# enoche/MMRec

Hardware: AMD Instinct MI355X
Metric: GCN-layer edges/sec (3-layer user-item CSR SpMM, d=64, fp32) (higher is better)
Workload: dtype f32

## Files before the change

include/mmrec_hip.h:

```cpp
#ifndef MMREC_HIP_H
#define MMREC_HIP_H

#include <stddef.h>
#include <stdint.h>

#ifdef __cplusplus
extern "C" {
#endif

#define MMREC_ABI_VERSION 16
#define MMREC_EMB_DIM 64

#define MMREC_ERR_BAD_ARG 10001
#define MMREC_ERR_UNSUPPORTED 10002

typedef void* mmrec_stream_t;

int mmrec_abi_version(void);
const char* mmrec_error_string(int err);

#ifndef MMREC_SPMM_CHUNK
#define MMREC_SPMM_CHUNK 512
#endif
#define MMREC_SPMM_LONG_ROW_DEFAULT 32

int mmrec_spmm_csr_f32(const int32_t* rowptr, const int32_t* colidx, const float* vals,
                       const float* X, float* Y, const float* Z, const float* acc_in, float* acc_out,
                       int32_t n_rows, int32_t d, float alpha, float beta, float acc_scale,
                       int32_t long_row_threshold, const int32_t* long_rows,
                       const int32_t* long_chunk_ptr, int32_t n_long, int32_t n_chunks,
                       float* partials, int32_t* long_tickets, mmrec_stream_t stream);

int mmrec_spmm_rows_f32(const int32_t* rowptr, const int32_t* colidx, const float* vals, const float* X,
                        const float* Z, int32_t z_compact, const int64_t* rows, int32_t n_list, int32_t d,
                        int32_t long_row_threshold, float* Y, mmrec_stream_t stream);
int mmrec_spmm_rows_any_f32(const int32_t* rowptr, const int32_t* colidx, const float* vals, const float* X,
                            const float* Z, int32_t z_compact, const int64_t* rows, int32_t n_list, int32_t d,
                            int32_t long_row_threshold, int32_t max_row_chunks, float* Y, mmrec_stream_t stream);
int mmrec_spmm_push_rows_f32(const int32_t* rowptr, const int32_t* colidx, const float* vals, const float* G,
                             float g_scale, const int64_t* rows, int32_t n_list, int32_t d, float* dX, float* dZ,
                             mmrec_stream_t stream);

int mmrec_spmm_csr_f32_layergcn(const int32_t* rowptr, const int32_t* colidx, const float* vals, const float* X,
                                float* Y, const float* ego, float* scaled, float* w, const float* acc_in,
                                float* acc_out, int32_t n_rows, int32_t d, int32_t long_row_threshold,
                                const int32_t* long_rows, const int32_t* long_chunk_ptr, int32_t n_long,
                                int32_t n_chunks, float* partials, int32_t* long_tickets, mmrec_stream_t stream);
int mmrec_spmm_csr_sched_f32(const int32_t* rowptr, const int32_t* colidx, const float* vals, const float* X, float* Y,
                             const float* Z, const float* acc_in, float* acc_out, int32_t n_rows, int32_t d, float alpha,
                             float beta, float acc_scale, int32_t long_row_threshold, const int32_t* long_rows,
                             const int32_t* long_chunk_ptr, int32_t n_long, int32_t n_chunks, float* partials,
                             int32_t* long_tickets, const int32_t* sched_row, const int32_t* sched_span,
                             const int32_t* sched_col, const float* sched_val, int32_t n_short, mmrec_stream_t stream);
int mmrec_spmm_csr_sched_f32_layergcn(const int32_t* rowptr, const int32_t* colidx, const float* vals, const float* X,
                                      float* Y, const float* ego, float* scaled, float* w, const float* acc_in,
                                      float* acc_out, int32_t n_rows, int32_t d, int32_t long_row_threshold,
                                      const int32_t* long_rows, const int32_t* long_chunk_ptr, int32_t n_long,
                                      int32_t n_chunks, float* partials, int32_t* long_tickets, const int32_t* sched_row,
                                      const int32_t* sched_span, const int32_t* sched_col, const float* sched_val,
                                      int32_t n_short, mmrec_stream_t stream);
int mmrec_spmm_row_keys(const int32_t* rowptr, const int32_t* colidx, const int32_t* col_degree, int32_t n_rows,
                        int32_t long_row_threshold, int32_t key_deg_max, int32_t* key, int32_t* key_degree,
                        mmrec_stream_t stream);

int mmrec_spmm_csr_masked_f32(const int32_t* rowptr, const int32_t* colidx, const float* vals, const float* X, float* Y,
                              const float* Z, const float* acc_in, float* acc_out, int32_t n_rows, int32_t d, float alpha,
                              float beta, float acc_scale, int32_t long_row_threshold, const int32_t* long_rows,
                              const int32_t* long_chunk_ptr, int32_t n_long, int32_t n_chunks, float* partials,
                              int32_t* long_tickets, const uint32_t* keep_bits, float val_scale, mmrec_stream_t stream);
int mmrec_edge_keep_bits(const uint8_t* keep, int64_t n_edges, const int64_t* perm_a, uint32_t* bits_a,
                         const int64_t* perm_b, uint32_t* bits_b, mmrec_stream_t stream);
int mmrec_spmm_plan_count(const int32_t* rowptr_host, int32_t n_rows, int32_t long_row_threshold,
                          int32_t* n_long, int32_t* n_chunks);
int mmrec_spmm_plan_fill(const int32_t* rowptr_host, int32_t n_rows, int32_t long_row_threshold,
                         int32_t* long_rows, int32_t* long_chunk_ptr);

int mmrec_cos_scale_fwd_f32(const float* E, const float* Ego, float* Out, float* w, float* acc,
                            int32_t n_rows, int32_t d, mmrec_stream_t stream);
int mmrec_cos_scale_bwd_f32(const float* dOut, const float* E, const float* Ego, const float* w,
                            float* dE, float* dEgo_accum, int32_t n_rows, int32_t d,
                            mmrec_stream_t stream);

#define MMREC_BPR_LOGSIG 0
#define MMREC_BPR_GAMMA 1

size_t mmrec_bpr_workspace_bytes(int32_t batch);
int mmrec_bpr_fwd_f32(const float* U, const float* P, const float* N, const int64_t* users,
                      const int64_t* pos, const int64_t* neg, int32_t batch, int32_t d,
                      int32_t variant, float scale, float* loss_out, float* coef, void* workspace,
                      mmrec_stream_t stream);
int mmrec_bpr_bwd_f32(const float* U, const float* P, const float* N, const int64_t* users,
                      const int64_t* pos, const int64_t* neg, int32_t batch, int32_t d,
                      const float* coef, const float* grad_scalar, float scale, float* dU, float* dP,
                      float* dN, mmrec_stream_t stream);

int mmrec_bpr_dots_f32(const float* U, const float* P, const float* N, const int64_t* users,
                       const int64_t* pos, const int64_t* neg, int32_t batch, int32_t d, float* dots,
                       mmrec_stream_t stream);
int mmrec_bpr_loss_from_dots_f32(const float* dots, int32_t batch, int32_t variant, float scale,
                                 float* loss_out, float* coef, void* workspace, mmrec_stream_t stream);

int mmrec_gather_sqnorm_fwd_f32(const float* E, const int64_t* ids, int32_t batch, int32_t d,
                                float* out, void* workspace, mmrec_stream_t stream);
int mmrec_gather_scale_add_bwd_f32(const float* E, const int64_t* ids, int32_t batch, int32_t d,
                                   const float* coef_scalar, float* dE, mmrec_stream_t stream);
#define MMREC_ROWS_REG_MAX_TERMS 6
size_t mmrec_rows_reg_workspace_bytes(int32_t n_terms, int32_t max_batch);
int mmrec_rows_reg_fwd_f32(const float* const* E, const int64_t* const* ids, const int32_t* batch, int32_t n_terms, int32_t d,
                           int32_t mode, float scale, float* out, float* coef, void* workspace, mmrec_stream_t stream);
int mmrec_rows_reg_bwd_f32(const float* const* E, const int64_t* const* ids, const int32_t* batch, int32_t n_terms, int32_t d,
                           const float* coef, const float* g, float* const* dE, mmrec_stream_t stream);

#define MMREC_BPR_MAX_TERMS 4
size_t mmrec_bpr_multi_workspace_bytes(int32_t n_terms, int32_t batch);
int mmrec_bpr_multi_fwd_f32(const float* U, const int64_t* users, const float* const* I, const int64_t* const* pos,
                            const int64_t* const* neg, const float* w, int32_t n_terms, int32_t batch, int32_t d, int32_t variant,
// ... 271 lines not shown
```

mmrec_amd/_lib.py:

```python
from __future__ import annotations

import ctypes
import os
from ctypes import c_char_p, c_float, c_int32, c_int64, c_size_t, c_uint64, c_void_p

import torch

_PKG = os.path.dirname(os.path.abspath(__file__))
LIB_PATH = os.environ.get("MMREC_HIP_LIB") or os.path.join(_PKG, "lib", "libmmrec_hip.so")
ABI_VERSION = 16

_P = c_void_p

SIGNATURES = {
    "mmrec_abi_version": (c_int32, []),
    "mmrec_error_string": (c_char_p, [c_int32]),
    "mmrec_spmm_csr_f32": (c_int32, [_P, _P, _P, _P, _P, _P, _P, _P, c_int32, c_int32, c_float,
                                     c_float, c_float, c_int32, _P, _P, c_int32, c_int32, _P, _P, _P]),
    "mmrec_spmm_csr_f32_layergcn": (c_int32, [_P, _P, _P, _P, _P, _P, _P, _P, _P, _P, c_int32, c_int32, c_int32,
                                              _P, _P, c_int32, c_int32, _P, _P, _P]),
    "mmrec_spmm_csr_sched_f32": (c_int32, [_P, _P, _P, _P, _P, _P, _P, _P, c_int32, c_int32, c_float,
                                           c_float, c_float, c_int32, _P, _P, c_int32, c_int32, _P, _P,
                                           _P, _P, _P, _P, c_int32, _P]),
    "mmrec_spmm_csr_sched_f32_layergcn": (c_int32, [_P, _P, _P, _P, _P, _P, _P, _P, _P, _P, c_int32, c_int32, c_int32,
                                                    _P, _P, c_int32, c_int32, _P, _P, _P, _P, _P, _P, c_int32, _P]),
    "mmrec_spmm_csr_masked_f32": (c_int32, [_P, _P, _P, _P, _P, _P, _P, _P, c_int32, c_int32, c_float,
                                            c_float, c_float, c_int32, _P, _P, c_int32, c_int32, _P, _P, _P, c_float, _P]),
    "mmrec_edge_keep_bits": (c_int32, [_P, c_int64, _P, _P, _P, _P, _P]),
    "mmrec_spmm_row_keys": (c_int32, [_P, _P, _P, c_int32, c_int32, c_int32, _P, _P, _P]),
    "mmrec_spmm_plan_count": (c_int32, [_P, c_int32, c_int32, _P, _P]),
    "mmrec_spmm_plan_fill": (c_int32, [_P, c_int32, c_int32, _P, _P]),
    "mmrec_cos_scale_fwd_f32": (c_int32, [_P, _P, _P, _P, _P, c_int32, c_int32, _P]),
    "mmrec_cos_scale_bwd_f32": (c_int32, [_P, _P, _P, _P, _P, _P, c_int32, c_int32, _P]),
    "mmrec_bpr_workspace_bytes": (c_size_t, [c_int32]),
    "mmrec_bpr_fwd_f32": (c_int32, [_P, _P, _P, _P, _P, _P, c_int32, c_int32, c_int32, c_float, _P,
                                    _P, _P, _P]),
    "mmrec_spmm_rows_f32": (c_int32, [_P, _P, _P, _P, _P, c_int32, _P, c_int32, c_int32, c_int32, _P, _P]),
    "mmrec_spmm_rows_any_f32": (c_int32, [_P, _P, _P, _P, _P, c_int32, _P, c_int32, c_int32, c_int32, c_int32, _P, _P]),
    "mmrec_spmm_push_rows_f32": (c_int32, [_P, _P, _P, _P, c_float, _P, c_int32, c_int32, _P, _P, _P]),
    "mmrec_bpr_dots_f32": (c_int32, [_P, _P, _P, _P, _P, _P, c_int32, c_int32, _P, _P]),
    "mmrec_bpr_loss_from_dots_f32": (c_int32, [_P, c_int32, c_int32, c_float, _P, _P, _P, _P]),
    "mmrec_bpr_bwd_f32": (c_int32, [_P, _P, _P, _P, _P, _P, c_int32, c_int32, _P, _P, c_float, _P, _P,
                                    _P, _P]),
    "mmrec_gather_sqnorm_fwd_f32": (c_int32, [_P, _P, c_int32, c_int32, _P, _P, _P]),
    "mmrec_gather_scale_add_bwd_f32": (c_int32, [_P, _P, c_int32, c_int32, _P, _P, _P]),
    "mmrec_infonce_workspace_bytes": (c_size_t, [c_int32]),
    "mmrec_infonce_fwd_f32": (c_int32, [_P, _P, _P, c_int32, c_int32, c_float, _P, _P, _P]),
    "mmrec_infonce_bwd_f32": (c_int32, [_P, c_int32, c_int32, c_float, _P, _P, _P, _P, _P]),
    "mmrec_linear_workspace_bytes": (c_size_t, [c_int32, c_int32, c_int32]),
    "mmrec_linear_fwd_f32": (c_int32, [_P, _P, _P, _P, c_int32, c_int32, c_int32, _P, _P]),
    "mmrec_linear_fwd_split_f32": (c_int32, [_P, _P, _P, _P, c_int32, c_int32, c_int32, _P, _P]),
    "mmrec_linear_bwd_split_workspace_bytes": (c_size_t, [c_int32, c_int32, c_int32]),
    "mmrec_linear_bwd_split_f32": (c_int32, [_P, _P, _P, _P, _P, _P, c_int32, c_int32, c_int32, _P, _P]),
    "mmrec_linear_bwd_w_f32": (c_int32, [_P, _P, _P, _P, c_int32, c_int32, c_int32, _P, _P]),
    "mmrec_linear_bwd_x_f32": (c_int32, [_P, _P, _P, c_int32, c_int32, c_int32, _P]),
    "mmrec_linear_rows_workspace_bytes": (c_size_t, [c_int32, c_int32, c_int32]),
    "mmrec_linear_rows_fwd_f32": (c_int32, [_P, c_int64, _P, _P, _P, _P, c_int32, c_int32, c_int32, c_int32, _P, _P]),
    "mmrec_linear_rows_bwd_f32": (c_int32, [_P, _P, c_int64, _P, _P, _P, _P, _P, c_int32, c_int32, c_int32, _P, _P]),
    "mmrec_edge_dot_f32": (c_int32, [_P, c_int64, _P, c_int64, _P, _P, c_int64, c_int32, _P, _P]),
    "mmrec_edge_dot_bwd_f32": (c_int32, [_P, _P, c_int64, _P, c_int64, _P, _P, c_int64, c_int32, _P, _P, _P]),
    "mmrec_segment_softmax_group_max": (c_int32, []),
    "mmrec_segment_softmax_f32": (c_int32, [_P, c_int32, _P, _P, c_int32, _P, c_int64, c_float, _P, _P]),
    "mmrec_segment_softmax_bwd_f32": (c_int32, [_P, c_int32, _P, _P, c_int32, _P, _P, c_int64, _P, _P]),
    "mmrec_edge_attention_group_max": (c_int32, []),
    "mmrec_edge_attention_f32": (c_int32, [_P, c_int32, _P, _P, _P, c_int32, _P, c_int64, _P, c_int64, c_int32, c_int64, c_float,
                                           _P, _P, _P]),
    "mmrec_edge_attention_bwd_f32": (c_int32, [_P, c_int32, _P, _P, _P, c_int32, _P, _P, _P, _P, c_int32, _P, c_int64, _P, c_int64,
                                               _P, _P, _P, _P, c_int32, c_int64, _P, _P, _P, _P, _P]),
    "mmrec_neighbor_max_group_max": (c_int32, []),
    "mmrec_neighbor_max_f32": (c_int32, [_P, c_int32, _P, _P, _P, c_int32, _P, c_int64, c_int32, c_int64, _P, _P, _P]),
    "mmrec_neighbor_max_bwd_f32": (c_int32, [_P, c_int32, _P, _P, _P, c_int32, _P, c_int64, _P, c_int32, c_int64, _P, _P, _P]),
    "mmrec_score_lse_split_cols": (c_int32, [c_int32, c_int32, c_int32]),
    "mmrec_score_lse_workspace_bytes": (c_size_t, [c_int32, c_int32, c_int32]),
    "mmrec_score_lse_f32": (c_int32, [_P, _P, c_int32, c_int32, c_int32, c_float, _P, _P, _P]),
    "mmrec_score_lse_bwd_f32": (c_int32, [_P, _P, c_int32, c_int32, c_int32, c_float, _P, _P, _P, _P, _P, _P]),
    "mmrec_hyper_rows_per_block": (c_int32, [c_int64]),
    "mmrec_hyper_workspace_bytes": (c_size_t, [c_int64, c_int64, c_int32]),
    "mmrec_hyper_assign_fwd_f32": (c_int32, [_P, _P, _P, c_int64, c_int32, c_float, c_float, _P, _P, _P]),
# ... 120 lines not shown
```

mmrec_amd/csrc/spmm.hip:

```cpp
#include "common.h"
#include "spmm_narrow.h"

#ifndef MMREC_SPMM_RPG
#define MMREC_SPMM_RPG(n_rows) ((n_rows) <= (1 << 18) ? 1 : 4)
#endif

namespace {

__device__ __forceinline__ void st_coherent(float4* p, float4 v) {
    unsigned long long* q = reinterpret_cast<unsigned long long*>(p);
    const unsigned long long lo = ((unsigned long long)__float_as_uint(v.y) << 32) | __float_as_uint(v.x);
    const unsigned long long hi = ((unsigned long long)__float_as_uint(v.w) << 32) | __float_as_uint(v.z);
    __hip_atomic_store(q, lo, __ATOMIC_RELAXED, __HIP_MEMORY_SCOPE_AGENT);
    __hip_atomic_store(q + 1, hi, __ATOMIC_RELAXED, __HIP_MEMORY_SCOPE_AGENT);
}
__device__ __forceinline__ float4 ld_coherent(const float4* p) {
    unsigned long long* q = reinterpret_cast<unsigned long long*>(const_cast<float4*>(p));
    const unsigned long long lo = __hip_atomic_load(q, __ATOMIC_RELAXED, __HIP_MEMORY_SCOPE_AGENT);
    const unsigned long long hi = __hip_atomic_load(q + 1, __ATOMIC_RELAXED, __HIP_MEMORY_SCOPE_AGENT);
    return make_float4(__uint_as_float((unsigned)lo), __uint_as_float((unsigned)(lo >> 32)),
                       __uint_as_float((unsigned)hi), __uint_as_float((unsigned)(hi >> 32)));
}

struct RowEpilogue {
    const float* Z;
    float* Y;
    const float* acc_in;
    float* acc_out;
    float alpha, beta, acc_scale;
    const float* ego;
    float* scaled;
    float* w_out;
};

struct RowSchedule {
    const int32_t* row;
    const int2* span;
    const int32_t* col;
    const float* val;
    int n_short;
};

template <int DCH, bool LG>
__device__ __forceinline__ void store_row(const RowEpilogue& ep, int row, int lane16, const float4 (&sum)[DCH]) {
    if (DCH == 1 && LG) {
        const size_t off = (size_t)row * 16 + lane16;
        const float4 y = f4_scale(ep.alpha, sum[0]);
        const float4 g = reinterpret_cast<const float4*>(ep.ego)[off];
        const float dot = row16_sum(f4_dot(y, g));
        const float ne = fmaxf(sqrtf(row16_sum(f4_dot(y, y))), 1e-8f);
        const float ng = fmaxf(sqrtf(row16_sum(f4_dot(g, g))), 1e-8f);
        const float w = dot / (ne * ng);
        const float4 o = f4_scale(w, y);
        if (ep.Y) reinterpret_cast<float4*>(ep.Y)[off] = y;
        reinterpret_cast<float4*>(ep.scaled)[off] = o;
        if (lane16 == 0) ep.w_out[row] = w;
        if (ep.acc_out)
            reinterpret_cast<float4*>(ep.acc_out)[off] =
                ep.acc_in ? f4_add(reinterpret_cast<const float4*>(ep.acc_in)[off], o) : o;
        return;
    }
#pragma unroll
    for (int ch = 0; ch < DCH; ++ch) {
        const size_t off = (size_t)row * (16 * DCH) + ch * 16 + lane16;
        float4 y = f4_scale(ep.alpha, sum[ch]);
        if (ep.Z) y = f4_fma(ep.beta, reinterpret_cast<const float4*>(ep.Z)[off], y);
        if (ep.Y) reinterpret_cast<float4*>(ep.Y)[off] = y;
        if (ep.acc_out) {
            const float4 a = reinterpret_cast<const float4*>(ep.acc_in)[off];
            reinterpret_cast<float4*>(ep.acc_out)[off] = f4_scale(ep.acc_scale, f4_add(a, y));
        }
    }
}

template <int DCH>
__device__ __forceinline__ void gather_span(const int32_t* __restrict__ colidx,
                                            const float* __restrict__ vals,
                                            const float4* __restrict__ X4, int s, int e, int lane16,
                                            float4 (&acc)[DCH]) {
    constexpr int NB = DCH == 1 ? 8 : (DCH <= 2 ? 4 : (DCH <= 4 ? 2 : 1));
    for (int base = s; base < e; base += 16) {
        const int k = base + lane16;
        int c = 0;
        float v = 0.f;
        if (k < e) {
            c = colidx[k];
            v = vals[k];
        }
        const int cnt = min(16, e - base);
        for (int j0 = 0; j0 < cnt; j0 += NB) {
            float4 x[NB][DCH];
            float vv[NB];
#pragma unroll
            for (int u = 0; u < NB; ++u) {
                const int j = j0 + u;
                const int cj = __shfl(c, j, 16);
                vv[u] = __shfl(v, j, 16);
#pragma unroll
                for (int ch = 0; ch < DCH; ++ch)
                    x[u][ch] = (j < cnt) ? X4[(size_t)cj * (16 * DCH) + ch * 16 + lane16] : f4_zero();
            }
#pragma unroll
            for (int u = 0; u < NB; ++u)
#pragma unroll
                for (int ch = 0; ch < DCH; ++ch) acc[ch] = f4_fma(vv[u], x[u][ch], acc[ch]);
        }
    }
}

template <int DCH, bool COHERENT, bool LG>
__device__ __forceinline__ void reduce_long_row(const float* __restrict__ partials, int c0, int c1, int row,
                                                const RowEpilogue& ep, float4 (*red)[16 * DCH]) {
    const int lane16 = threadIdx.x & 15, g = threadIdx.x >> 4;
#pragma unroll
    for (int ch = 0; ch < DCH; ++ch) {
        float4 t = f4_zero();
        for (int c = c0 + g; c < c1; c += 16) {
            const float4* src = reinterpret_cast<const float4*>(partials) + (size_t)c * (16 * DCH) + ch * 16 + lane16;
            t = f4_add(t, COHERENT ? ld_coherent(src) : *src);
        }
        red[g][ch * 16 + lane16] = t;
    }
    __syncthreads();
    if (g == 0) {
        float4 r[DCH];
#pragma unroll
        for (int ch = 0; ch < DCH; ++ch) {
            r[ch] = red[0][ch * 16 + lane16];
#pragma unroll
            for (int k = 1; k < 16; ++k) r[ch] = f4_add(r[ch], red[k][ch * 16 + lane16]);
        }
        store_row<DCH, LG>(ep, row, lane16, r);
    }
}

template <int DCH, bool LG, bool SCHED>
__global__ __launch_bounds__(256) void spmm_rows_kernel(
    const int32_t* __restrict__ rowptr, const int32_t* __restrict__ colidx,
    const float* __restrict__ vals, const float* __restrict__ X, RowEpilogue ep, int n_rows,
    int long_t, int rows_per_group, const int32_t* __restrict__ long_rows,
    const int32_t* __restrict__ long_chunk_ptr, int n_long, int n_chunks,
    float* __restrict__ partials, int32_t* __restrict__ tickets, RowSchedule sched) {
    __shared__ float4 red[16][16 * DCH];
    __shared__ int s_last;
    const int lane16 = threadIdx.x & 15;
    const int g = threadIdx.x >> 4;
    const float4* X4 = reinterpret_cast<const float4*>(X);
    if ((int)blockIdx.x < n_chunks) {
        const int chunk = blockIdx.x;
        int lo = 0, hi = n_long;
        while (hi - lo > 1) {
            const int mid = (lo + hi) >> 1;
            if (long_chunk_ptr[mid] <= chunk) lo = mid; else hi = mid;
        }
        const int row = long_rows[lo];
        const int cs = rowptr[row] + (chunk - long_chunk_ptr[lo]) * MMREC_SPMM_CHUNK;
        const int ce = min(cs + MMREC_SPMM_CHUNK, rowptr[row + 1]);
        float4 acc[DCH];
#pragma unroll
        for (int ch = 0; ch < DCH; ++ch) acc[ch] = f4_zero();
        for (int base = cs + g * 16; base < ce; base += 256)
            gather_span<DCH>(colidx, vals, X4, base, min(base + 16, ce), lane16, acc);
#pragma unroll
        for (int ch = 0; ch < DCH; ++ch) red[g][ch * 16 + lane16] = acc[ch];
        __syncthreads();
        if (g == 0) {
            float4 t[DCH];
#pragma unroll
            for (int ch = 0; ch < DCH; ++ch) {
                t[ch] = red[0][ch * 16 + lane16];
#pragma unroll
                for (int i = 1; i < 16; ++i) t[ch] = f4_add(t[ch], red[i][ch * 16 + lane16]);
            }
            if (long_chunk_ptr[lo + 1] - long_chunk_ptr[lo] == 1) {
                store_row<DCH, LG>(ep, row, lane16, t);
            } else {
#pragma unroll
                for (int ch = 0; ch < DCH; ++ch) {
                    float4* dst = reinterpret_cast<float4*>(partials) + (size_t)chunk * (16 * DCH) + ch * 16 + lane16;
                    if (tickets) st_coherent(dst, t[ch]); else *dst = t[ch];
                }
            }
        }
        const int c0 = long_chunk_ptr[lo], c1 = long_chunk_ptr[lo + 1];
        if (!tickets || c1 - c0 == 1) return;
        if (threadIdx.x < 64) {
            __atomic_signal_fence(__ATOMIC_SEQ_CST);
            __builtin_amdgcn_s_waitcnt(0);
            __atomic_signal_fence(__ATOMIC_SEQ_CST);
            __builtin_amdgcn_fence(__ATOMIC_RELEASE, "workgroup");
            if (threadIdx.x == 0)
                s_last = __hip_atomic_fetch_add(tickets + lo, 1, __ATOMIC_RELAXED, __HIP_MEMORY_SCOPE_AGENT) == c1 - c0 - 1;
        }
        __syncthreads();
        if (!s_last) return;
        __builtin_amdgcn_fence(__ATOMIC_ACQUIRE, "workgroup");
        reduce_long_row<DCH, true, LG>(partials, c0, c1, row, ep, red);
        if (threadIdx.x == 0) __hip_atomic_store(tickets + lo, 0, __ATOMIC_RELAXED, __HIP_MEMORY_SCOPE_AGENT);
        return;
    }
    if (SCHED) {
        const int slot0 = ((int)blockIdx.x - n_chunks) * 16 * rows_per_group + g;
#pragma unroll 1
        for (int i = 0; i < rows_per_group; ++i) {
            const int slot = slot0 + i * 16;
            if (slot >= sched.n_short) break;
            const int row = sched.row[slot];
            const int2 se = sched.span[slot];
            float4 acc[DCH];
#pragma unroll
            for (int ch = 0; ch < DCH; ++ch) acc[ch] = f4_zero();
            gather_span<DCH>(sched.col, sched.val, X4, se.x, se.y, lane16, acc);
            store_row<DCH, LG>(ep, row, lane16, acc);
        }
        return;
    }
    const int row0 = ((int)blockIdx.x - n_chunks) * 16 * rows_per_group + g;
#pragma unroll 1
    for (int i = 0; i < rows_per_group; ++i) {
        const int row = row0 + i * 16;
        if (row >= n_rows) break;
        const int s = rowptr[row], e = rowptr[row + 1];
        if (e - s > long_t) continue;
        float4 acc[DCH];
#pragma unroll
        for (int ch = 0; ch < DCH; ++ch) acc[ch] = f4_zero();
        gather_span<DCH>(colidx, vals, X4, s, e, lane16, acc);
        store_row<DCH, LG>(ep, row, lane16, acc);
    }
}

template <int DCH, bool LG>
__global__ __launch_bounds__(256) void spmm_long_reduce_kernel(
    const int32_t* __restrict__ long_rows, const int32_t* __restrict__ long_chunk_ptr, int n_long,
    const float* __restrict__ partials, RowEpilogue ep) {
    __shared__ float4 red[16][16 * DCH];
    const int i = blockIdx.x;
    const int c0 = long_chunk_ptr[i], c1 = long_chunk_ptr[i + 1];
    if (c1 - c0 <= 1) return;
    reduce_long_row<DCH, false, LG>(partials, c0, c1, long_rows[i], ep, red);
}

template <int DCH, bool LG = false, bool SCHED = false>
void launch_spmm(hipStream_t s, int blocks, int nch, const int32_t* rowptr, const int32_t* colidx,
                 const float* vals, const float* X, const RowEpilogue& ep, int n_rows, int long_t,
                 int rows_per_group, const int32_t* long_rows, const int32_t* long_chunk_ptr, int n_long,
                 float* partials, int32_t* tickets, const RowSchedule& sched = RowSchedule{}) {
    if (blocks + nch > 0)
        hipLaunchKernelGGL((spmm_rows_kernel<DCH, LG, SCHED>), dim3(blocks + nch), dim3(256), 0, s, rowptr, colidx, vals, X,
                           ep, n_rows, long_t, rows_per_group, long_rows, long_chunk_ptr, n_long, nch, partials, tickets,
                           sched);
    if (!tickets && n_long > 0 && nch > n_long)
        hipLaunchKernelGGL((spmm_long_reduce_kernel<DCH, LG>), dim3(n_long), dim3(256), 0, s, long_rows,
                           long_chunk_ptr, n_long, partials, ep);
}

template <int DCH>
__device__ __forceinline__ void gather_span_masked(const int32_t* __restrict__ colidx, const float* __restrict__ vals,
                                                   const uint32_t* __restrict__ keep_bits, float val_scale,
                                                   const float4* __restrict__ X4, int s, int e, int lane16,
                                                   float4 (&acc)[DCH]) {
    constexpr int NB = DCH == 1 ? 8 : (DCH <= 2 ? 4 : (DCH <= 4 ? 2 : 1));
    const int gshift = threadIdx.x & 48;
    for (int base = s; base < e; base += 16) {
        const int k = base + lane16;
        int c = 0;
        float v = 0.f;
        bool kept = false;
        if (k < e) {
            kept = (keep_bits[k >> 5] >> (k & 31)) & 1u;
            c = colidx[k];
            v = vals[k] * val_scale;
        }
        unsigned m = (unsigned)(__ballot(kept) >> gshift) & 0xffffu;
        while (m) {
            float4 x[NB][DCH];
            float vv[NB];
#pragma unroll
            for (int u = 0; u < NB; ++u) {
                const bool on = m != 0;
                const int j = on ? __ffs(m) - 1 : 0;
                m &= m - 1;
                const int cj = __shfl(c, j, 16);
                const float vj = __shfl(v, j, 16);
                vv[u] = on ? vj : 0.f;
#pragma unroll
                for (int ch = 0; ch < DCH; ++ch)
                    x[u][ch] = on ? X4[(size_t)cj * (16 * DCH) + ch * 16 + lane16] : f4_zero();
            }
#pragma unroll
            for (int u = 0; u < NB; ++u)
#pragma unroll
                for (int ch = 0; ch < DCH; ++ch) acc[ch] = f4_fma(vv[u], x[u][ch], acc[ch]);
        }
    }
}

template <int DCH>
__global__ __launch_bounds__(256) void spmm_rows_masked_kernel(
    const int32_t* __restrict__ rowptr, const int32_t* __restrict__ colidx, const float* __restrict__ vals,
    const uint32_t* __restrict__ keep_bits, float val_scale, const float* __restrict__ X, RowEpilogue ep, int n_rows,
    int long_t, int rows_per_group, const int32_t* __restrict__ long_rows, const int32_t* __restrict__ long_chunk_ptr,
    int n_long, int n_chunks, float* __restrict__ partials, int32_t* __restrict__ tickets) {
    __shared__ float4 red[16][16 * DCH];
    __shared__ int s_last;
    const int lane16 = threadIdx.x & 15;
// ... 356 lines not shown
    if (n_long > 0 && (!long_rows || !long_chunk_ptr || !partials || n_chunks <= 0))
        return MMREC_ERR_BAD_ARG;
    if (!sched_args_ok(sched_row, sched_span, sched_col, sched_val, n_short, n_rows)) return MMREC_ERR_BAD_ARG;
    if (Y == X || acc_out == X) return MMREC_ERR_BAD_ARG;
    RowEpilogue ep{Z, Y, acc_in, acc_out, alpha, Z ? beta : 0.f, acc_scale, nullptr, nullptr, nullptr};
    const RowSchedule sched{sched_row, reinterpret_cast<const int2*>(sched_span), sched_col, sched_val, n_short};
    hipStream_t s = mmrec_stream(stream);
    const int rows_per_group = MMREC_SPMM_RPG(n_rows);
    const int blocks = (n_short + 16 * rows_per_group - 1) / (16 * rows_per_group);
    const int long_t = n_long > 0 ? long_row_threshold : INT32_MAX;
    const int nch = n_long > 0 ? n_chunks : 0;
    int32_t* tickets = n_long > 0 ? long_tickets : nullptr;
#define MMREC_SPMM_CASE(D)                                                                                      \
    case D:                                                                                                     \
        launch_spmm<D, false, true>(s, blocks, nch, rowptr, colidx, vals, X, ep, n_rows, long_t, rows_per_group, \
                                    long_rows, long_chunk_ptr, n_long, partials, tickets, sched);               \
        break;
    switch (d / MMREC_EMB_DIM) {
        MMREC_SPMM_CASE(1) MMREC_SPMM_CASE(2) MMREC_SPMM_CASE(3) MMREC_SPMM_CASE(4) MMREC_SPMM_CASE(5)
        MMREC_SPMM_CASE(6)
    }
#undef MMREC_SPMM_CASE
    MMREC_RETURN_LAUNCH_STATUS();
}

extern "C" int mmrec_spmm_csr_sched_f32_layergcn(const int32_t* rowptr, const int32_t* colidx, const float* vals,
                                                 const float* X, float* Y, const float* ego, float* scaled, float* w,
                                                 const float* acc_in, float* acc_out, int32_t n_rows, int32_t d,
                                                 int32_t long_row_threshold, const int32_t* long_rows,
                                                 const int32_t* long_chunk_ptr, int32_t n_long, int32_t n_chunks,
                                                 float* partials, int32_t* long_tickets, const int32_t* sched_row,
                                                 const int32_t* sched_span, const int32_t* sched_col,
                                                 const float* sched_val, int32_t n_short, mmrec_stream_t stream) {
    if (d != MMREC_EMB_DIM) return MMREC_ERR_UNSUPPORTED;
    if (n_rows < 0 || n_long < 0 || n_chunks < 0 || long_row_threshold < 0) return MMREC_ERR_BAD_ARG;
    if (n_rows == 0) return 0;
    if (!rowptr || !X || !ego || !scaled || !w) return MMREC_ERR_BAD_ARG;
    if (n_long > 0 && (!long_rows || !long_chunk_ptr || !partials || n_chunks <= 0)) return MMREC_ERR_BAD_ARG;
    if (!sched_args_ok(sched_row, sched_span, sched_col, sched_val, n_short, n_rows)) return MMREC_ERR_BAD_ARG;
    if (Y == X || scaled == X || acc_out == X) return MMREC_ERR_BAD_ARG;
    RowEpilogue ep{nullptr, Y, acc_in, acc_out, 1.f, 0.f, 1.f, ego, scaled, w};
    const RowSchedule sched{sched_row, reinterpret_cast<const int2*>(sched_span), sched_col, sched_val, n_short};
    hipStream_t s = mmrec_stream(stream);
    const int rows_per_group = MMREC_SPMM_RPG(n_rows);
    const int blocks = (n_short + 16 * rows_per_group - 1) / (16 * rows_per_group);
    const int long_t = n_long > 0 ? long_row_threshold : INT32_MAX;
    const int nch = n_long > 0 ? n_chunks : 0;
    int32_t* tickets = n_long > 0 ? long_tickets : nullptr;
    launch_spmm<1, true, true>(s, blocks, nch, rowptr, colidx, vals, X, ep, n_rows, long_t, rows_per_group, long_rows,
                               long_chunk_ptr, n_long, partials, tickets, sched);
    MMREC_RETURN_LAUNCH_STATUS();
}

extern "C" int mmrec_spmm_row_keys(const int32_t* rowptr, const int32_t* colidx, const int32_t* col_degree,
                                   int32_t n_rows, int32_t long_row_threshold, int32_t key_deg_max, int32_t* key,
                                   int32_t* key_degree, mmrec_stream_t stream) {
    if (n_rows < 0 || long_row_threshold < 0 || key_deg_max < 0) return MMREC_ERR_BAD_ARG;
    if (n_rows == 0) return 0;
    if (!rowptr || !colidx || !col_degree || !key || !key_degree) return MMREC_ERR_BAD_ARG;
    hipLaunchKernelGGL(spmm_row_keys_kernel, dim3((n_rows + 15) / 16), dim3(256), 0, mmrec_stream(stream), rowptr, colidx,
                       col_degree, n_rows, long_row_threshold, key_deg_max, key, key_degree);
    MMREC_RETURN_LAUNCH_STATUS();
}

extern "C" int mmrec_spmm_plan_count(const int32_t* rowptr_host, int32_t n_rows,
                                     int32_t long_row_threshold, int32_t* n_long, int32_t* n_chunks) {
    if (!rowptr_host || !n_long || !n_chunks || n_rows < 0) return MMREC_ERR_BAD_ARG;
    int32_t nl = 0, nc = 0;
    for (int32_t r = 0; r < n_rows; ++r) {
        const int32_t deg = rowptr_host[r + 1] - rowptr_host[r];
        if (deg > long_row_threshold) {
            ++nl;
            nc += (deg + MMREC_SPMM_CHUNK - 1) / MMREC_SPMM_CHUNK;
        }
    }
    *n_long = nl;
    *n_chunks = nc;
    return 0;
}

extern "C" int mmrec_spmm_plan_fill(const int32_t* rowptr_host, int32_t n_rows,
                                    int32_t long_row_threshold, int32_t* long_rows,
                                    int32_t* long_chunk_ptr) {
    if (!rowptr_host || !long_rows || !long_chunk_ptr || n_rows < 0) return MMREC_ERR_BAD_ARG;
    int32_t nl = 0, nc = 0;
    for (int32_t r = 0; r < n_rows; ++r) {
        const int32_t deg = rowptr_host[r + 1] - rowptr_host[r];
        if (deg > long_row_threshold) {
            long_rows[nl] = r;
            long_chunk_ptr[nl] = nc;
            ++nl;
            nc += (deg + MMREC_SPMM_CHUNK - 1) / MMREC_SPMM_CHUNK;
        }
    }
    long_chunk_ptr[nl] = nc;
    return 0;
}

extern "C" int mmrec_cos_scale_fwd_f32(const float* E, const float* Ego, float* Out, float* w,
                                       float* acc, int32_t n_rows, int32_t d, mmrec_stream_t stream) {
    if (d != MMREC_EMB_DIM) return MMREC_ERR_UNSUPPORTED;
    if (n_rows < 0 || (n_rows > 0 && (!E || !Ego || !Out || !w))) return MMREC_ERR_BAD_ARG;
    if (n_rows == 0) return 0;
    hipLaunchKernelGGL(cos_scale_fwd_kernel, dim3((n_rows + 15) / 16), dim3(256), 0,
                       mmrec_stream(stream), E, Ego, Out, w, acc, n_rows);
    MMREC_RETURN_LAUNCH_STATUS();
// ... 14 lines not shown
```

mmrec_amd/hip_ops.py:

```python
from __future__ import annotations

import ctypes
import math

import numpy as np
import torch

from . import _lib

EMB_DIM = 64
LINEAR_F16X3_DEFAULT = True
LINEAR_F16X3 = LINEAR_F16X3_DEFAULT
SLICE_WIDTHS = (8, 16, 32)
SPMM_CHUNK = 512
LONG_ROW_DEFAULT = None


def default_long_row_threshold(n_cols):
    import os
    forced = os.environ.get("MMREC_LONG_ROW_THRESHOLD")
    if forced:
        return int(forced)
    return 16 if n_cols <= (1 << 18) else 32

# ... 300 lines not shown
    def __init__(self, g: CsrGraph, reorder, n_left=None):
        if g.n_rows != g.n_cols:
            raise _lib.MMRecHipError("PermutedGraph needs a square graph")
        dev, n = g.rowptr.device, g.n_rows
        idx, val = g.to_coo_host()
        perm = locality_order(g.rowptr_host, idx[1], n, reorder, n_left=n_left)
        self.base, self.reorder = g, reorder
        self.perm = torch.from_numpy(perm).to(dev)
        inv = np.empty(n, dtype=np.int64)
        inv[perm] = np.arange(n, dtype=np.int64)
        self.inv = torch.from_numpy(inv).to(dev)
        self.graph = CsrGraph.from_coo_host(np.stack([perm[idx[0]], perm[idx[1]]]), val, n, n, dev, symmetric=g.symmetric,
                                            long_row_threshold=g.long_row_threshold)
        self.n_rows = self.n_cols = n
        self.nnz = g.nnz

    def to_new(self, X):
        return X.index_select(0, self.inv)

    def to_old(self, Xp):
        return Xp.index_select(0, self.perm)


def spmm_raw(g: CsrGraph, X, Y=None, Z=None, acc_in=None, acc_out=None, alpha=1.0, beta=1.0,
             acc_scale=1.0):
    lib = _lib.load()
    _chk(X, torch.float32, "X", 2)
    d = X.shape[1]
    if (d not in SLICE_WIDTHS and (d % EMB_DIM or d > 6 * EMB_DIM)) or X.shape[0] < g.n_cols:
        raise _lib.MMRecHipError("X must be [>=%d, 64*k <= 384 (or a feature slice of 8 / 16 / 32 columns)], got %s" %
                                 (g.n_cols, tuple(X.shape)))
    for t, nm in ((Y, "Y"), (Z, "Z"), (acc_in, "acc_in"), (acc_out, "acc_out")):
        if t is not None:
            _chk(t, torch.float32, nm, 2)
            if t.shape[0] < g.n_rows or t.shape[1] != d:
                raise _lib.MMRecHipError("%s must be [>=%d, %d]" % (nm, g.n_rows, d))
    sc = g.scheduled(d)
    if sc is not None:
        g.checked(lib.mmrec_spmm_csr_sched_f32(_p(g.rowptr), _p(g.colidx), _p(g.vals), _p(X), _p(Y), _p(Z),
                                               _p(acc_in), _p(acc_out), g.n_rows, d, float(alpha),
                                               float(beta), float(acc_scale), g.long_row_threshold,
                                               _p(g.long_rows), _p(g.long_chunk_ptr), g.n_long, g.n_chunks,
                                               _p(g.partials_for(d)), _p(g.long_tickets), _p(sc["row"]), _p(sc["span"]),
                                               _p(sc["col"]), _p(sc["val"]), sc["n_short"], _stream()), "spmm_csr_sched_f32")
        return Y if Y is not None else acc_out
    g.checked(lib.mmrec_spmm_csr_f32(_p(g.rowptr), _p(g.colidx), _p(g.vals), _p(X), _p(Y), _p(Z),
                                     _p(acc_in), _p(acc_out), g.n_rows, d, float(alpha),
                                     float(beta), float(acc_scale), g.long_row_threshold,
                                     _p(g.long_rows), _p(g.long_chunk_ptr), g.n_long, g.n_chunks,
                                     _p(g.partials_for(d)), _p(g.long_tickets), _stream()), "spmm_csr_f32")
    return Y if Y is not None else acc_out


ROWS_MAX_CHUNKS = 480


def rows_servable(g: CsrGraph, d):
    if d not in SLICE_WIDTHS + (EMB_DIM,):
        return False
    return g.n_chunks == g.n_long or (d == EMB_DIM and g.max_row_chunks <= ROWS_MAX_CHUNKS)


def spmm_rows_raw(g: CsrGraph, X, rows, Z=None, z_compact=False):
    lib = _lib.load()
    _chk(X, torch.float32, "X", 2), _chk(rows, torch.int64, "rows", 1)
    d = X.shape[1]
    if not rows_servable(g, d) or X.shape[0] < g.n_cols:
        raise _lib.MMRecHipError("spmm_rows: graph with multi-chunk rows, or X not [>=%d, 8 / 16 / 32 / 64]" % g.n_cols)
    if Z is not None and (_chk(Z, torch.float32, "Z", 2).shape[0] < (rows.numel() if z_compact else g.n_rows) or Z.shape[1] != d):
        raise _lib.MMRecHipError("Z must be [>=%d, %d]" % (rows.numel() if z_compact else g.n_rows, d))
    Y = torch.empty(rows.numel(), d, dtype=torch.float32, device=X.device)
    long_t = g.long_row_threshold if g.n_long > 0 else 2 ** 31 - 1
    if g.n_chunks == g.n_long:
        _lib.check(lib.mmrec_spmm_rows_f32(_p(g.rowptr), _p(g.colidx), _p(g.vals), _p(X), _p(Z), 1 if z_compact else 0, _p(rows),
                                           rows.numel(), d, long_t, _p(Y), _stream()), "spmm_rows_f32")
    else:
        _lib.check(lib.mmrec_spmm_rows_any_f32(_p(g.rowptr), _p(g.colidx), _p(g.vals), _p(X), _p(Z), 1 if z_compact else 0, _p(rows),
                                               rows.numel(), d, long_t, g.max_row_chunks, _p(Y), _stream()), "spmm_rows_any_f32")
    return Y


def spmm_push_rows_raw(g: CsrGraph, G, rows, dX=None, dZ=None, scale=1.0):
    lib = _lib.load()
    _chk(G, torch.float32, "G", 2), _chk(rows, torch.int64, "rows", 1)
    d = G.shape[1]
    if G.shape[0] != rows.numel() or d not in SLICE_WIDTHS + (EMB_DIM,):
        raise _lib.MMRecHipError("G must be [len(rows), 8 / 16 / 32 / 64]")
    for t, nm, n in ((dX, "dX", g.n_cols), (dZ, "dZ", g.n_rows)):
        if t is not None and (_chk(t, torch.float32, nm, 2).shape[0] < n or t.shape[1] != d):
            raise _lib.MMRecHipError("%s must be [>=%d, %d]" % (nm, n, d))
    _lib.check(lib.mmrec_spmm_push_rows_f32(_p(g.rowptr), _p(g.colidx), _p(g.vals), _p(G), float(scale), _p(rows), rows.numel(),
                                            d, _p(dX), _p(dZ), _stream()), "spmm_push_rows_f32")


class _SpmmRows(torch.autograd.Function):

    @staticmethod
    def forward(ctx, X, Z_rows, g, rows):
        ctx.g, ctx.x_shape, ctx.has_z = g, tuple(X.shape), Z_rows is not None
        ctx.save_for_backward(rows)
        return spmm_rows_raw(g, X.contiguous(), rows, None if Z_rows is None else Z_rows.contiguous(), z_compact=True)

    @staticmethod
    def backward(ctx, dY):
        rows, = ctx.saved_tensors
        dY = dY.contiguous()
# ... 4 lines not shown
        return dX, (dY if ctx.has_z and ctx.needs_input_grad[1] else None), None, None


def spmm_rows(g: CsrGraph, X, rows, Z_rows=None):
    if DETERMINISTIC or isinstance(g, PermutedGraph) or not rows_servable(g, X.shape[1]):
        out = spmm(g, X).index_select(0, rows)
        return out if Z_rows is None else out + Z_rows
    return _SpmmRows.apply(X, Z_rows, g, rows)


class _SpMM(torch.autograd.Function):
    @staticmethod
    def forward(ctx, X, Z, g):
        ctx.g, ctx.has_z, ctx.x_rows = g, Z is not None, X.shape[0]
        X = X.contiguous()
        Y = torch.empty(g.n_rows, X.shape[1], dtype=torch.float32, device=X.device)
        spmm_raw(g, X, Y=Y, Z=None if Z is None else Z.contiguous(), beta=1.0)
        return Y

    @staticmethod
    def backward(ctx, dY):
        dY = dY.contiguous()
        gt = ctx.g.transpose()
        dX = None
        if ctx.needs_input_grad[0]:
            alloc = torch.empty if ctx.x_rows == gt.n_rows else torch.zeros
            dX = alloc(ctx.x_rows, dY.shape[1], dtype=torch.float32, device=dY.device)
            spmm_raw(gt, dY, Y=dX)
        return dX, (dY if ctx.has_z and ctx.needs_input_grad[1] else None), None


def spmm(g: CsrGraph, X, Z=None):
    if isinstance(g, PermutedGraph):
        out = spmm(g.graph, g.to_new(X), None if Z is None else g.to_new(Z))
        return g.to_old(out)
    d = X.shape[1]
    if d % EMB_DIM and d not in SLICE_WIDTHS:
        pad = EMB_DIM - d % EMB_DIM
        Xp = torch.nn.functional.pad(X, (0, pad))
        Zp = None if Z is None else torch.nn.functional.pad(Z, (0, pad))
        return _SpMM.apply(Xp, Zp, g)[:, :d]
    return _SpMM.apply(X, Z, g)


class _LightGCNMean(torch.autograd.Function):

    @staticmethod
    def forward(ctx, E0, g, n_layers):
        ctx.g, ctx.L = g, int(n_layers)
        E0 = E0.contiguous()
        L = ctx.L
        if L == 0:
            return E0.clone()
        acc = torch.empty_like(E0)
        bufs = [torch.empty_like(E0) if L > 1 else None, torch.empty_like(E0) if L > 2 else None]
        cur = E0
        for layer in range(1, L + 1):
            last = layer == L
            Y = None if last else bufs[(layer - 1) % 2]
            spmm_raw(g, cur, Y=Y, acc_in=E0 if layer == 1 else acc, acc_out=acc,
                     acc_scale=1.0 / (L + 1) if last else 1.0)
            cur = Y
        return acc

    @staticmethod
    def backward(ctx, dOut):
        L, gt = ctx.L, ctx.g.transpose()
        dOut = dOut.contiguous()
        if L == 0:
            return dOut, None, None
        s = 1.0 / (L + 1)
        bufs = [torch.empty_like(dOut), torch.empty_like(dOut) if L > 1 else None]
        t = dOut
        for j in range(L):
            out = bufs[j % 2]
            spmm_raw(gt, t, Y=out, Z=dOut, alpha=s if j == 0 else 1.0, beta=s)
            t = out
        return t, None, None


def lightgcn_mean(g, E0, n_layers):
    if isinstance(g, PermutedGraph):
        return g.to_old(_LightGCNMean.apply(g.to_new(E0), g.graph, n_layers))
    return _LightGCNMean.apply(E0, g, n_layers)


def row_blocks_of_one_buffer(ts):
    if any(t is None or not t.is_contiguous() or t.dtype != ts[0].dtype for t in ts):
        return False
    base = ts[0].untyped_storage().data_ptr()
    end = ts[0].data_ptr()
    for t in ts:
        if t.untyped_storage().data_ptr() != base or t.data_ptr() != end:
            return False
        end += t.numel() * t.element_size()
    return end <= base + ts[0].untyped_storage().nbytes()


class _LightGCNMeanParts(torch.autograd.Function):

    @staticmethod
    def forward(ctx, g, n_layers, *parts):
        ctx.sizes = [p.shape[0] for p in parts]
        if row_blocks_of_one_buffer(parts):
            E0 = parts[0].detach().as_strided((sum(ctx.sizes), parts[0].shape[1]), (parts[0].shape[1], 1))
        else:
            E0 = torch.cat([p.detach() for p in parts], dim=0)
        ctx.g, ctx.L = g, int(n_layers)
        out = _LightGCNMean.forward(ctx, E0, g, n_layers)
        return tuple(out.split(ctx.sizes))

    @staticmethod
    def backward(ctx, *grads):
        like = next(x for x in grads if x is not None)
        n, d = sum(ctx.sizes), like.shape[1]
        if row_blocks_of_one_buffer(grads):
            dOut = grads[0].as_strided((n, d), (d, 1))
        else:
            dOut = torch.empty((n, d), dtype=like.dtype, device=like.device)
            for dst, src in zip(dOut.split(ctx.sizes), grads):
                dst.zero_() if src is None else dst.copy_(src)
        t = _LightGCNMean.backward(ctx, dOut)[0]
        return (None, None) + tuple(t.split(ctx.sizes))


def lightgcn_mean_parts(g: CsrGraph, parts, n_layers):
    return _LightGCNMeanParts.apply(g, n_layers, *parts)


ROWS_LAST_LAYER = True


class _LightGCNMeanPartsRows(torch.autograd.Function):

    @staticmethod
    def forward(ctx, g, n_layers, rows, *parts):
        ctx.sizes = [p.shape[0] for p in parts]
        if row_blocks_of_one_buffer(parts):
            E0 = parts[0].detach().as_strided((sum(ctx.sizes), parts[0].shape[1]), (parts[0].shape[1], 1))
        else:
            E0 = torch.cat([p.detach() for p in parts], dim=0)
        ctx.save_for_backward(rows)
        L = int(n_layers)
        if L >= 1 and ROWS_LAST_LAYER and rows_servable(g, E0.shape[1]) and E0.shape[0] == g.n_rows == g.n_cols:
            ctx.g, ctx.L = g, L
            E0 = E0.contiguous()
            cur, acc = E0, E0
            if L > 1:
                acc = torch.empty_like(E0)
                bufs = [torch.empty_like(E0), torch.empty_like(E0) if L > 2 else None]
                for layer in range(1, L):
                    Y = bufs[(layer - 1) % 2]
                    spmm_raw(g, cur, Y=Y, acc_in=E0 if layer == 1 else acc, acc_out=acc, acc_scale=1.0)
                    cur = Y
            return spmm_rows_raw(g, cur, rows, Z=acc) * (1.0 / (L + 1))
        out = _LightGCNMean.forward(ctx, E0, g, n_layers)
        return out.index_select(0, rows)

    @staticmethod
    def backward(ctx, dRows):
        rows, = ctx.saved_tensors
        L, g = ctx.L, ctx.g
        dRows = dRows.contiguous()
        n, d = sum(ctx.sizes), dRows.shape[1]
        s = 1.0 / (L + 1)
        t = torch.zeros((n, d), dtype=dRows.dtype, device=dRows.device)
        if L == 0:
            spmm_push_rows_raw(g, dRows, rows, dZ=t)
            return (None, None, None) + tuple(t.split(ctx.sizes))
        spmm_push_rows_raw(g, dRows, rows, dX=t, dZ=t, scale=s)
        gt = g.transpose()
        for _ in range(1, L):
            out = torch.empty_like(t)
            spmm_raw(gt, t, Y=out)
            spmm_push_rows_raw(g, dRows, rows, dZ=out, scale=s)
            t = out
        return (None, None, None) + tuple(t.split(ctx.sizes))


class _MeanPartsRowsThenItemRows(torch.autograd.Function):

    @staticmethod
    def forward(ctx, g, n_layers, rows, mm, item_rows, b, user_table, item_table):
        import types
        inner = types.SimpleNamespace(saved=None)
        inner.save_for_backward = lambda *t: setattr(inner, 'saved', t)
        at = _LightGCNMeanPartsRows.forward(inner, g, n_layers, rows, user_table, item_table)
        ia = spmm_rows_raw(mm, item_table.detach().contiguous(), item_rows, at[b:].contiguous(), z_compact=True)
        ctx.inner = types.SimpleNamespace(sizes=inner.sizes, g=inner.g, L=inner.L)
        ctx.mm, ctx.b = mm, int(b)
        ctx.save_for_backward(rows, item_rows)
        return at[:b].contiguous(), ia

    @staticmethod
    def backward(ctx, d_user_rows, d_ia):
        rows, item_rows = ctx.saved_tensors
        inner = ctx.inner
        inner.saved_tensors = (rows,)
        d_ia = d_ia.contiguous()
        d_rows = torch.cat((d_user_rows.contiguous(), d_ia), dim=0)
# ... 2232 lines not shown
```

Before: 31.26 billion.

## Defer LightGCN layer-sum accumulation to a final multi-table SpMM epilogue

Adds a layer-sum epilogue for the d=64 SpMM kernels. Instead of reading and writing an accumulator on every layer, the intermediate layers now write only Y, and the last layer's kernel sums up to four saved layer tables plus its own result into the output. In the row-gather path, the tables are summed only for the requested rows. The aim is to cut the per-layer read-modify-write accumulator traffic. In exchange the final layer reads more tables and more intermediate buffers are allocated.

```diff
diff --git a/include/mmrec_hip.h b/include/mmrec_hip.h
--- a/include/mmrec_hip.h
+++ b/include/mmrec_hip.h
@@ -62,6 +62,21 @@
 int mmrec_spmm_row_keys(const int32_t* rowptr, const int32_t* colidx, const int32_t* col_degree, int32_t n_rows,
                         int32_t long_row_threshold, int32_t key_deg_max, int32_t* key, int32_t* key_degree,
                         mmrec_stream_t stream);
+
+int mmrec_spmm_csr_layersum_f32(const int32_t* rowptr, const int32_t* colidx, const float* vals, const float* X, float* Y,
+                                const float* S0, const float* S1, const float* S2, const float* S3, int32_t n_sum,
+                                float* out, int32_t n_rows, int32_t d, float alpha, float acc_scale,
+                                int32_t long_row_threshold, const int32_t* long_rows, const int32_t* long_chunk_ptr,
+                                int32_t n_long, int32_t n_chunks, float* partials, int32_t* long_tickets,
+                                mmrec_stream_t stream);
+int mmrec_spmm_csr_sched_layersum_f32(const int32_t* rowptr, const int32_t* colidx, const float* vals, const float* X,
+                                      float* Y, const float* S0, const float* S1, const float* S2, const float* S3,
+                                      int32_t n_sum, float* out, int32_t n_rows, int32_t d, float alpha, float acc_scale,
+                                      int32_t long_row_threshold, const int32_t* long_rows,
+                                      const int32_t* long_chunk_ptr, int32_t n_long, int32_t n_chunks, float* partials,
+                                      int32_t* long_tickets, const int32_t* sched_row, const int32_t* sched_span,
+                                      const int32_t* sched_col, const float* sched_val, int32_t n_short,
+                                      mmrec_stream_t stream);
 
 int mmrec_spmm_csr_masked_f32(const int32_t* rowptr, const int32_t* colidx, const float* vals, const float* X, float* Y,
                               const float* Z, const float* acc_in, float* acc_out, int32_t n_rows, int32_t d, float alpha,
diff --git a/mmrec_amd/_lib.py b/mmrec_amd/_lib.py
--- a/mmrec_amd/_lib.py
+++ b/mmrec_amd/_lib.py
@@ -24,6 +24,11 @@
                                            _P, _P, _P, _P, c_int32, _P]),
     "mmrec_spmm_csr_sched_f32_layergcn": (c_int32, [_P, _P, _P, _P, _P, _P, _P, _P, _P, _P, c_int32, c_int32, c_int32,
                                                     _P, _P, c_int32, c_int32, _P, _P, _P, _P, _P, _P, c_int32, _P]),
+    "mmrec_spmm_csr_layersum_f32": (c_int32, [_P, _P, _P, _P, _P, _P, _P, _P, _P, c_int32, _P, c_int32, c_int32, c_float,
+                                              c_float, c_int32, _P, _P, c_int32, c_int32, _P, _P, _P]),
+    "mmrec_spmm_csr_sched_layersum_f32": (c_int32, [_P, _P, _P, _P, _P, _P, _P, _P, _P, c_int32, _P, c_int32, c_int32, c_float,
+                                                    c_float, c_int32, _P, _P, c_int32, c_int32, _P, _P,
+                                                    _P, _P, _P, _P, c_int32, _P]),
     "mmrec_spmm_csr_masked_f32": (c_int32, [_P, _P, _P, _P, _P, _P, _P, _P, c_int32, c_int32, c_float,
                                             c_float, c_float, c_int32, _P, _P, c_int32, c_int32, _P, _P, _P, c_float, _P]),
     "mmrec_edge_keep_bits": (c_int32, [_P, c_int64, _P, _P, _P, _P, _P]),
diff --git a/mmrec_amd/csrc/spmm.hip b/mmrec_amd/csrc/spmm.hip
--- a/mmrec_amd/csrc/spmm.hip
+++ b/mmrec_amd/csrc/spmm.hip
@@ -73,6 +73,30 @@
     }
 }
 
+struct LayerSumEpilogue {
+    const float* S0;
+    const float* S1;
+    const float* S2;
+    const float* S3;
+    int n_sum;
+    float* Y;
+    float* out;
+    float alpha, acc_scale;
+};
+
+template <int DCH, bool LG>
+__device__ __forceinline__ void store_row(const LayerSumEpilogue& ep, int row, int lane16, const float4 (&sum)[DCH]) {
+    static_assert(DCH == 1 && !LG, "the layer-sum epilogue is a d = 64 form");
+    const size_t off = (size_t)row * 16 + lane16;
+    const float4 y = f4_scale(ep.alpha, sum[0]);
+    if (ep.Y) reinterpret_cast<float4*>(ep.Y)[off] = y;
+    float4 t = reinterpret_cast<const float4*>(ep.S0)[off];
+    if (ep.n_sum > 1) t = f4_add(t, reinterpret_cast<const float4*>(ep.S1)[off]);
+    if (ep.n_sum > 2) t = f4_add(t, reinterpret_cast<const float4*>(ep.S2)[off]);
+    if (ep.n_sum > 3) t = f4_add(t, reinterpret_cast<const float4*>(ep.S3)[off]);
+    reinterpret_cast<float4*>(ep.out)[off] = f4_scale(ep.acc_scale, f4_add(t, y));
+}
+
 template <int DCH>
 __device__ __forceinline__ void gather_span(const int32_t* __restrict__ colidx,
                                             const float* __restrict__ vals,
@@ -108,9 +132,9 @@
     }
 }
 
-template <int DCH, bool COHERENT, bool LG>
+template <int DCH, bool COHERENT, bool LG, class EP>
 __device__ __forceinline__ void reduce_long_row(const float* __restrict__ partials, int c0, int c1, int row,
-                                                const RowEpilogue& ep, float4 (*red)[16 * DCH]) {
+                                                const EP& ep, float4 (*red)[16 * DCH]) {
     const int lane16 = threadIdx.x & 15, g = threadIdx.x >> 4;
 #pragma unroll
     for (int ch = 0; ch < DCH; ++ch) {
@@ -134,10 +158,10 @@
     }
 }
 
-template <int DCH, bool LG, bool SCHED>
+template <int DCH, bool LG, bool SCHED, class EP = RowEpilogue>
 __global__ __launch_bounds__(256) void spmm_rows_kernel(
     const int32_t* __restrict__ rowptr, const int32_t* __restrict__ colidx,
-    const float* __restrict__ vals, const float* __restrict__ X, RowEpilogue ep, int n_rows,
+    const float* __restrict__ vals, const float* __restrict__ X, EP ep, int n_rows,
     int long_t, int rows_per_group, const int32_t* __restrict__ long_rows,
     const int32_t* __restrict__ long_chunk_ptr, int n_long, int n_chunks,
     float* __restrict__ partials, int32_t* __restrict__ tickets, RowSchedule sched) {
@@ -230,10 +254,10 @@
     }
 }
 
-template <int DCH, bool LG>
+template <int DCH, bool LG, class EP = RowEpilogue>
 __global__ __launch_bounds__(256) void spmm_long_reduce_kernel(
     const int32_t* __restrict__ long_rows, const int32_t* __restrict__ long_chunk_ptr, int n_long,
-    const float* __restrict__ partials, RowEpilogue ep) {
+    const float* __restrict__ partials, EP ep) {
     __shared__ float4 red[16][16 * DCH];
     const int i = blockIdx.x;
     const int c0 = long_chunk_ptr[i], c1 = long_chunk_ptr[i + 1];
@@ -241,17 +265,17 @@
     reduce_long_row<DCH, false, LG>(partials, c0, c1, long_rows[i], ep, red);
 }
 
-template <int DCH, bool LG = false, bool SCHED = false>
+template <int DCH, bool LG = false, bool SCHED = false, class EP = RowEpilogue>
 void launch_spmm(hipStream_t s, int blocks, int nch, const int32_t* rowptr, const int32_t* colidx,
-                 const float* vals, const float* X, const RowEpilogue& ep, int n_rows, int long_t,
+                 const float* vals, const float* X, const EP& ep, int n_rows, int long_t,
                  int rows_per_group, const int32_t* long_rows, const int32_t* long_chunk_ptr, int n_long,
                  float* partials, int32_t* tickets, const RowSchedule& sched = RowSchedule{}) {
     if (blocks + nch > 0)
-        hipLaunchKernelGGL((spmm_rows_kernel<DCH, LG, SCHED>), dim3(blocks + nch), dim3(256), 0, s, rowptr, colidx, vals, X,
+        hipLaunchKernelGGL((spmm_rows_kernel<DCH, LG, SCHED, EP>), dim3(blocks + nch), dim3(256), 0, s, rowptr, colidx, vals, X,
                            ep, n_rows, long_t, rows_per_group, long_rows, long_chunk_ptr, n_long, nch, partials, tickets,
                            sched);
     if (!tickets && n_long > 0 && nch > n_long)
-        hipLaunchKernelGGL((spmm_long_reduce_kernel<DCH, LG>), dim3(n_long), dim3(256), 0, s, long_rows,
+        hipLaunchKernelGGL((spmm_long_reduce_kernel<DCH, LG, EP>), dim3(n_long), dim3(256), 0, s, long_rows,
                            long_chunk_ptr, n_long, partials, ep);
 }
 
@@ -714,6 +738,70 @@
     MMREC_RETURN_LAUNCH_STATUS();
 }
 
+namespace {
+int layersum_args(const float* const (&S)[4], int32_t n_sum, int32_t d, const float* X, const float* Y, const float* out) {
+    if (d != MMREC_EMB_DIM || n_sum < 1 || n_sum > 4 || !out) return MMREC_ERR_BAD_ARG;
+    for (int k = 0; k < n_sum; ++k)
+        if (!S[k]) return MMREC_ERR_BAD_ARG;
+    if (Y == X || out == X || out == Y) return MMREC_ERR_BAD_ARG;
+    return 0;
+}
+}
+
+extern "C" int mmrec_spmm_csr_layersum_f32(const int32_t* rowptr, const int32_t* colidx, const float* vals,
+                                           const float* X, float* Y, const float* S0, const float* S1,
+                                           const float* S2, const float* S3, int32_t n_sum, float* out,
+                                           int32_t n_rows, int32_t d, float alpha, float acc_scale,
+                                           int32_t long_row_threshold, const int32_t* long_rows,
+                                           const int32_t* long_chunk_ptr, int32_t n_long, int32_t n_chunks,
+                                           float* partials, int32_t* long_tickets, mmrec_stream_t stream) {
+    if (n_rows < 0 || n_long < 0 || n_chunks < 0 || long_row_threshold < 0) return MMREC_ERR_BAD_ARG;
+    const float* const S[4] = {S0, S1, S2, S3};
+    if (const int rc = layersum_args(S, n_sum, d, X, Y, out)) return rc;
+    if (n_rows == 0) return 0;
+    if (!rowptr || !X) return MMREC_ERR_BAD_ARG;
+    if (n_long > 0 && (!long_rows || !long_chunk_ptr || !partials || n_chunks <= 0)) return MMREC_ERR_BAD_ARG;
+    const LayerSumEpilogue ep{S0, S1, S2, S3, n_sum, Y, out, alpha, acc_scale};
+    hipStream_t s = mmrec_stream(stream);
+    const int rows_per_group = MMREC_SPMM_RPG(n_rows);
+    const int blocks = (n_rows + 16 * rows_per_group - 1) / (16 * rows_per_group);
+    const int long_t = n_long > 0 ? long_row_threshold : INT32_MAX;
+    const int nch = n_long > 0 ? n_chunks : 0;
+    int32_t* tickets = n_long > 0 ? long_tickets : nullptr;
+    launch_spmm<1, false, false>(s, blocks, nch, rowptr, colidx, vals, X, ep, n_rows, long_t, rows_per_group, long_rows,
+                                long_chunk_ptr, n_long, partials, tickets);
+    MMREC_RETURN_LAUNCH_STATUS();
+}
+
+extern "C" int mmrec_spmm_csr_sched_layersum_f32(const int32_t* rowptr, const int32_t* colidx, const float* vals,
+                                                 const float* X, float* Y, const float* S0, const float* S1,
+                                                 const float* S2, const float* S3, int32_t n_sum, float* out,
+                                                 int32_t n_rows, int32_t d, float alpha, float acc_scale,
+                                                 int32_t long_row_threshold, const int32_t* long_rows,
+                                                 const int32_t* long_chunk_ptr, int32_t n_long, int32_t n_chunks,
+                                                 float* partials, int32_t* long_tickets, const int32_t* sched_row,
+                                                 const int32_t* sched_span, const int32_t* sched_col,
+                                                 const float* sched_val, int32_t n_short, mmrec_stream_t stream) {
+    if (n_rows < 0 || n_long < 0 || n_chunks < 0 || long_row_threshold < 0) return MMREC_ERR_BAD_ARG;
+    const float* const S[4] = {S0, S1, S2, S3};
+    if (const int rc = layersum_args(S, n_sum, d, X, Y, out)) return rc;
+    if (n_rows == 0) return 0;
+    if (!rowptr || !X) return MMREC_ERR_BAD_ARG;
+    if (n_long > 0 && (!long_rows || !long_chunk_ptr || !partials || n_chunks <= 0)) return MMREC_ERR_BAD_ARG;
+    if (!sched_args_ok(sched_row, sched_span, sched_col, sched_val, n_short, n_rows)) return MMREC_ERR_BAD_ARG;
+    const LayerSumEpilogue ep{S0, S1, S2, S3, n_sum, Y, out, alpha, acc_scale};
+    const RowSchedule sched{sched_row, reinterpret_cast<const int2*>(sched_span), sched_col, sched_val, n_short};
+    hipStream_t s = mmrec_stream(stream);
+    const int rows_per_group = MMREC_SPMM_RPG(n_rows);
+    const int blocks = (n_short + 16 * rows_per_group - 1) / (16 * rows_per_group);
+    const int long_t = n_long > 0 ? long_row_threshold : INT32_MAX;
+    const int nch = n_long > 0 ? n_chunks : 0;
+    int32_t* tickets = n_long > 0 ? long_tickets : nullptr;
+    launch_spmm<1, false, true>(s, blocks, nch, rowptr, colidx, vals, X, ep, n_rows, long_t, rows_per_group, long_rows,
+                               long_chunk_ptr, n_long, partials, tickets, sched);
+    MMREC_RETURN_LAUNCH_STATUS();
+}
+
 extern "C" int mmrec_spmm_row_keys(const int32_t* rowptr, const int32_t* colidx, const int32_t* col_degree,
                                    int32_t n_rows, int32_t long_row_threshold, int32_t key_deg_max, int32_t* key,
                                    int32_t* key_degree, mmrec_stream_t stream) {
diff --git a/mmrec_amd/hip_ops.py b/mmrec_amd/hip_ops.py
--- a/mmrec_amd/hip_ops.py
+++ b/mmrec_amd/hip_ops.py
@@ -376,6 +376,60 @@
     return Y if Y is not None else acc_out
 
 
+LAYER_SUM_MAX_TABLES = 4
+
+
+def spmm_layersum_raw(g: CsrGraph, X, tables, out, Y=None, alpha=1.0, acc_scale=1.0):
+    lib = _lib.load()
+    _chk(X, torch.float32, "X", 2)
+    d = X.shape[1]
+    if d != EMB_DIM or X.shape[0] < g.n_cols or not 1 <= len(tables) <= LAYER_SUM_MAX_TABLES:
+        raise _lib.MMRecHipError("layer sum: X must be [>=%d, 64] with 1 .. 4 tables, got %s and %d" %
+                                 (g.n_cols, tuple(X.shape), len(tables)))
+    for t, nm in [(out, "out")] + ([(Y, "Y")] if Y is not None else []) + [(t, "S%d" % i) for i, t in enumerate(tables)]:
+        if _chk(t, torch.float32, nm, 2).shape[0] < g.n_rows or t.shape[1] != d:
+            raise _lib.MMRecHipError("%s must be [>=%d, %d]" % (nm, g.n_rows, d))
+    S = [_p(t) for t in tables] + [None] * (LAYER_SUM_MAX_TABLES - len(tables))
+    sc = g.scheduled(d)
+    if sc is not None:
+        g.checked(lib.mmrec_spmm_csr_sched_layersum_f32(_p(g.rowptr), _p(g.colidx), _p(g.vals), _p(X), _p(Y), S[0], S[1], S[2],
+                                                        S[3], len(tables), _p(out), g.n_rows, d, float(alpha),
+                                                        float(acc_scale), g.long_row_threshold, _p(g.long_rows),
+                                                        _p(g.long_chunk_ptr), g.n_long, g.n_chunks, _p(g.partials_for(d)),
+                                                        _p(g.long_tickets), _p(sc["row"]), _p(sc["span"]), _p(sc["col"]),
+                                                        _p(sc["val"]), sc["n_short"], _stream()), "spmm_csr_sched_layersum_f32")
+        return out
+    g.checked(lib.mmrec_spmm_csr_layersum_f32(_p(g.rowptr), _p(g.colidx), _p(g.vals), _p(X), _p(Y), S[0], S[1], S[2], S[3],
+                                              len(tables), _p(out), g.n_rows, d, float(alpha), float(acc_scale),
+                                              g.long_row_threshold, _p(g.long_rows), _p(g.long_chunk_ptr), g.n_long,
+                                              g.n_chunks, _p(g.partials_for(d)), _p(g.long_tickets), _stream()),
+              "spmm_csr_layersum_f32")
+    return out
+
+
+LAYER_SUM_AT_END = True
+LAYER_SUM_MAX_LAYERS = 5
+
+
+def _layer_sum_at_end(d, L):
+    return LAYER_SUM_AT_END and d == EMB_DIM and 1 <= L <= LAYER_SUM_MAX_LAYERS
+
+
+def _layers_before_last(g, E0, L):
+    cur, tables = E0, [E0]
+    for layer in range(1, L):
+        Y = torch.empty_like(E0)
+        if L - layer >= LAYER_SUM_MAX_TABLES:
+            acc = torch.empty_like(E0)
+            spmm_raw(g, cur, Y=Y, acc_in=tables[0], acc_out=acc, acc_scale=1.0)
+            tables = [acc]
+        else:
+            spmm_raw(g, cur, Y=Y)
+            tables.append(Y)
+        cur = Y
+    return cur, tables
+
+
 ROWS_MAX_CHUNKS = 480
 
 
@@ -486,6 +540,9 @@
         L = ctx.L
         if L == 0:
             return E0.clone()
+        if _layer_sum_at_end(E0.shape[1], L):
+            cur, tables = _layers_before_last(g, E0, L)
+            return spmm_layersum_raw(g, cur, tables, torch.empty_like(E0), acc_scale=1.0 / (L + 1))
         acc = torch.empty_like(E0)
         bufs = [torch.empty_like(E0) if L > 1 else None, torch.empty_like(E0) if L > 2 else None]
         cur = E0
@@ -580,6 +637,12 @@
             ctx.g, ctx.L = g, L
             E0 = E0.contiguous()
             cur, acc = E0, E0
+            if _layer_sum_at_end(E0.shape[1], L):
+                cur, tables = _layers_before_last(g, E0, L)
+                z = tables[0].index_select(0, rows)
+                for t in tables[1:]:
+                    z = z + t.index_select(0, rows)
+                return spmm_rows_raw(g, cur, rows, Z=z, z_compact=True) * (1.0 / (L + 1))
             if L > 1:
                 acc = torch.empty_like(E0)
                 bufs = [torch.empty_like(E0), torch.empty_like(E0) if L > 2 else None]
```

Result: no change. 31.29 billion, median of 2 (+0.1%).
